# bcollico/Deep-Multiview-Depth-Estimation

Hardware: AMD Instinct MI355X
Metric: depth maps/sec + warp-kernel HBM GB/s, 3-view 640x512 D=192, 1/2/4/8 GPU (higher is better)
Workload: dtype f32

## Files before the change

deep-multiview-depth-estimation_amd/csrc/conv3d_narrow.hip:

```cpp
#include <algorithm>

#include "launchers.h"
#include "packed.h"

namespace mvs {
namespace {

constexpr int kTX = 32, kTY = 8, kDT = 4;

struct Head1 {
  const float* w1p;
  const float *sc, *sh, *mu;
  float* y1;
  int o0[3], on[3];
  int pad[3];
};

#ifndef MVS_HEAD_WAVES
#define MVS_HEAD_WAVES 3
#endif

template <int COUT, int C4, bool WZ = false, int DT = kDT, bool FOLD = false, bool C1 = false>
__global__ __launch_bounds__(kBlock) __attribute__((amdgpu_waves_per_eu(C1 ? MVS_HEAD_WAVES : 1)))
void conv3d_k3_narrow_kernel(
    const float* __restrict__ in, const float* __restrict__ wt, float* __restrict__ out, int Cin,
    int D, int H, int W, int tiles_x, int tiles_y, int dgroups, int n_batch, const float* __restrict__ bn_scale,
    const float* __restrict__ bn_shift, const float* __restrict__ bn_mean, const float* __restrict__ in2,
    const float* __restrict__ ibn, Head1 h1) {
  static_assert(!FOLD || (COUT == 1 && C4 == 0), "folded input BN: conv_out on NCDHW");
  static_assert(!WZ || DT == 4, "depth Winograd: two windows of 2");
  static_assert(!C1 || (COUT == 8 && C4 == 1 && WZ), "fused conv_1_0: the fp32 conv_0_0 kernel");
  constexpr int kPX = kTX + 2, kPY = kTY + 2, kPD = DT + 2;
  constexpr int kPlane = kPX * kPY;
  constexpr int kStage = kPD * kPlane;
  constexpr int kPer = (kStage + kBlock - 1) / kBlock;
  constexpr int NP = COUT / 2;
  constexpr int NQ = C4 ? 4 : 1;
  __shared__ float lds[NQ * kStage];
  __shared__ __attribute__((aligned(16))) float w1s[C1 ? 27 * 16 * 4 : 4];
  const int total = (int)gridDim.x;
  int t = xcd_work_id((int)blockIdx.x, total);
  if (t >= tiles_x * tiles_y * dgroups * n_batch) return;
  const int tx0 = (t % tiles_x) * kTX;
  t /= tiles_x;
  const int ty0 = (t % tiles_y) * kTY;
  t /= tiles_y;
  const int d0 = (t % dgroups) * DT;
  const int b = t / dgroups;
  const size_t plane = (size_t)H * W;
  const size_t vol = (size_t)D * plane;
  const float* ib = in + (size_t)b * Cin * vol;
  const uint2* ib16 = reinterpret_cast<const uint2*>(reinterpret_cast<const char*>(in) + (size_t)b * Cin * vol * 2);

  int goff[kPer];
  bool gok[kPer];
#pragma unroll
  for (int j = 0; j < kPer; ++j) {
    const int e = (int)threadIdx.x + j * kBlock;
    const int pd = e / kPlane, r = e % kPlane;
    const int py = r / kPX, px = r % kPX;
    const int gz = d0 + pd - 1, gy = ty0 + py - 1, gx = tx0 + px - 1;
    gok[j] = e < kStage && gz >= 0 && gz < D && gy >= 0 && gy < H && gx >= 0 && gx < W;
    goff[j] = gok[j] ? (int)((size_t)gz * plane + (size_t)gy * W + gx) : 0;
  }
  float pre[kPer][NQ];
  float pre2[FOLD ? kPer : 1];
  const float* ib2 = FOLD ? in2 + (size_t)b * Cin * vol : nullptr;
  auto fetch = [&](int q) {
    if constexpr (C4 == 2) {
      const uint2* src = ib16 + (size_t)q * vol;
#pragma unroll
      for (int j = 0; j < kPer; ++j) {
        const uint2 v = gok[j] ? src[goff[j]] : make_uint2(0u, 0u);
        pre[j][0] = __uint_as_float(v.x << 16);
        pre[j][1] = __uint_as_float(v.x & 0xFFFF0000u);
        pre[j][2] = __uint_as_float(v.y << 16);
        pre[j][3] = __uint_as_float(v.y & 0xFFFF0000u);
      }
    } else if constexpr (C4) {
      const float4* src = reinterpret_cast<const float4*>(ib) + (size_t)q * vol;
#pragma unroll
      for (int j = 0; j < kPer; ++j) {
        const float4 v = gok[j] ? src[goff[j]] : make_float4(0.0f, 0.0f, 0.0f, 0.0f);
        pre[j][0] = v.x;
        pre[j][1] = v.y;
        pre[j][2] = v.z;
        pre[j][3] = v.w;
      }
    } else {
      const float* src = ib + (size_t)q * vol;
#pragma unroll
      for (int j = 0; j < kPer; ++j) pre[j][0] = gok[j] ? src[goff[j]] : 0.0f;
      if constexpr (FOLD) {
        const float* src2 = ib2 + (size_t)q * vol;
#pragma unroll
        for (int j = 0; j < kPer; ++j) pre2[j] = gok[j] ? src2[goff[j]] : 0.0f;
      }
    }
  };
  fetch(0);

  const int lx = (int)threadIdx.x % kTX, ly = (int)threadIdx.x / kTX;
  f2v acc2[DT][NP > 0 ? NP : 1];
  float acc1[DT];
#pragma unroll
  for (int d = 0; d < DT; ++d) {
    acc1[d] = 0.0f;
#pragma unroll
    for (int q = 0; q < (NP > 0 ? NP : 1); ++q) acc2[d][q] = f2v{0.0f, 0.0f};
  }
  f2v accw[WZ ? 2 : 1][WZ ? 4 : 1][WZ ? NP : 1];
  if constexpr (WZ) {
#pragma unroll
    for (int a = 0; a < 2; ++a)
#pragma unroll
      for (int ps = 0; ps < 4; ++ps)
#pragma unroll
        for (int q = 0; q < NP; ++q) accw[a][ps][q] = f2v{0.0f, 0.0f};
  }
  const int c1lane = (int)threadIdx.x & 63, c1wave = (int)threadIdx.x >> 6;
  const int m16 = c1lane & 15, kq = c1lane >> 4;
  f4v c1acc[2] = {f4v{0.0f, 0.0f, 0.0f, 0.0f}, f4v{0.0f, 0.0f, 0.0f, 0.0f}};
  int abase[2] = {0, 0};
  if constexpr (C1) {
#pragma unroll
    for (int rb = 0; rb < 2; ++rb) {
      const int rbi = 2 * c1wave + rb, wy = rbi & 3, wzz = rbi >> 2;
      abase[rb] = kq * kStage + (2 * wzz) * kPlane + (2 * wy) * kPX + 2 * m16;
    }
  }

  const int passes = C4 ? Cin / 4 : Cin;
  for (int q = 0; q < passes; ++q) {
    __syncthreads();
    if constexpr (FOLD) {
      const float sa = ibn[q], ha = ibn[Cin + q], ma = ibn[2 * Cin + q];
      const float sb = ibn[3 * Cin + q], hb = ibn[4 * Cin + q], mb = ibn[5 * Cin + q];
#pragma unroll
      for (int j = 0; j < kPer; ++j)
        if (gok[j]) pre[j][0] = fmaxf((pre[j][0] - ma) * sa + ha, 0.0f) + fmaxf((pre2[j] - mb) * sb + hb, 0.0f);
    }
#pragma unroll
    for (int j = 0; j < kPer; ++j) {
      const int e = (int)threadIdx.x + j * kBlock;
      if (e < kStage)
#pragma unroll
        for (int u = 0; u < NQ; ++u) lds[u * kStage + e] = pre[j][u];
    }
    if constexpr (C1) {
      const f4v* src = reinterpret_cast<const f4v*>(h1.w1p) + (size_t)q * 432;
      f4v* dst = reinterpret_cast<f4v*>(w1s);
      for (int i = (int)threadIdx.x; i < 432; i += kBlock) dst[i] = src[i];
    }
    __syncthreads();
    if (q + 1 < passes) fetch(q + 1);
#pragma unroll 1
    for (int u = 0; u < NQ; ++u) {
      const int c = q * NQ + u;
      const float* lc = lds + u * kStage;
      if constexpr (WZ) {
#pragma unroll
        for (int ky = 0; ky < 3; ++ky)
#pragma unroll
          for (int kx = 0; kx < 3; ++kx) {
            float t[kPD];
#pragma unroll
            for (int p = 0; p < kPD; ++p) t[p] = lc[p * kPlane + (ly + ky) * kPX + lx + kx];
            const f2v z0 = {t[0], t[2]}, z1 = {t[1], t[3]}, z2 = {t[2], t[4]}, z3 = {t[3], t[5]};
            const f2v v[4] = {z0 - z2, z1 + z2, z2 - z1, z1 - z3};
            asm volatile("" ::: "memory");
            const f2v* wg = reinterpret_cast<const f2v*>(wt + ((size_t)(c * 9 + ky * 3 + kx) * 4) * 8);
#pragma unroll
            for (int ps = 0; ps < 4; ++ps)
#pragma unroll
              for (int qq = 0; qq < NP; ++qq) {
                const f2v u = wg[ps * 4 + qq];
                accw[0][ps][qq] = __builtin_elementwise_fma(f2v{v[ps].x, v[ps].x}, u, accw[0][ps][qq]);
                accw[1][ps][qq] = __builtin_elementwise_fma(f2v{v[ps].y, v[ps].y}, u, accw[1][ps][qq]);
              }
          }
        continue;
      }
      float tap[kPD][3][3];
#pragma unroll
      for (int p = 0; p < kPD; ++p)
#pragma unroll
        for (int ry = 0; ry < 3; ++ry)
#pragma unroll
          for (int kx = 0; kx < 3; ++kx) tap[p][ry][kx] = lc[p * kPlane + (ly + ry) * kPX + lx + kx];
#pragma unroll
      for (int kd = 0; kd < 3; ++kd) {
        if constexpr (COUT == 8) {
#pragma unroll
          for (int qq = 0; qq < NP; ++qq) {
            asm volatile("" ::: "memory");
            const f2v* wg = reinterpret_cast<const f2v*>(wt + ((size_t)(c * 3 + kd) * 9) * 8) + qq;
            f2v wp[9];
#pragma unroll
            for (int k = 0; k < 9; ++k) wp[k] = wg[k * 4];
#pragma unroll
            for (int d = 0; d < DT; ++d)
#pragma unroll
              for (int ky = 0; ky < 3; ++ky)
#pragma unroll
                for (int kx = 0; kx < 3; ++kx) {
                  const float tv = tap[d + kd][ky][kx];
                  acc2[d][qq] = __builtin_elementwise_fma(f2v{tv, tv}, wp[ky * 3 + kx], acc2[d][qq]);
                }
          }
        } else {
          asm volatile("" ::: "memory");
          const float* wg = wt + ((size_t)c * 3 + kd) * 9;
          float w9[9];
#pragma unroll
          for (int k = 0; k < 9; ++k) w9[k] = wg[k];
#pragma unroll
          for (int d = 0; d < DT; ++d)
#pragma unroll
            for (int ky = 0; ky < 3; ++ky)
#pragma unroll
              for (int kx = 0; kx < 3; ++kx) acc1[d] = fmaf(tap[d + kd][ky][kx], w9[ky * 3 + kx], acc1[d]);
        }
      }
    }
    if constexpr (C1) {
#pragma unroll
      for (int t = 0; t < 27; ++t) {
        const int tz = t / 9, ty = (t / 3) % 3, tx = t % 3;
        const float bv = w1s[t * 64 + m16 * 4 + kq];
#pragma unroll
        for (int rb = 0; rb < 2; ++rb)
          c1acc[rb] = __builtin_amdgcn_mfma_f32_16x16x4f32(lds[abase[rb] + tz * kPlane + ty * kPX + tx], bv,
                                                           c1acc[rb], 0, 0, 0);
      }
    }
  }

  if constexpr (C1) {
    const float sc = h1.sc ? h1.sc[m16] : 1.0f, sh = h1.sc ? h1.sh[m16] : 0.0f, mu = h1.sc ? h1.mu[m16] : 0.0f;
#pragma unroll
    for (int rb = 0; rb < 2; ++rb) {
      const int rbi = 2 * c1wave + rb, wy = rbi & 3, wzz = rbi >> 2;
      const int oz = (d0 - 1 + 2 * wzz + h1.pad[0]) >> 1, oy = (ty0 - 1 + 2 * wy + h1.pad[1]) >> 1;
      if (oz < h1.o0[0] || oz >= h1.o0[0] + h1.on[0] || oy < h1.o0[1] || oy >= h1.o0[1] + h1.on[1]) continue;
#pragma unroll
      for (int r = 0; r < 4; ++r) {
        const int ox = (tx0 - 1 + 2 * (4 * kq + r) + h1.pad[2]) >> 1;
        if (ox < h1.o0[2] || ox >= h1.o0[2] + h1.on[2]) continue;
        float v = c1acc[rb][r];
        if (h1.sc) v = fmaxf((v - mu) * sc + sh, 0.0f);
        h1.y1[((((size_t)b * h1.on[0] + (oz - h1.o0[0])) * h1.on[1] + (oy - h1.o0[1])) * h1.on[2] + (ox - h1.o0[2])) *
                  16 + m16] = v;
      }
    }
  }

  if constexpr (WZ) {
#pragma unroll
    for (int a = 0; a < 2; ++a)
#pragma unroll
      for (int qq = 0; qq < NP; ++qq) {
        acc2[2 * a][qq] = accw[a][0][qq] + accw[a][1][qq] + accw[a][2][qq];
        acc2[2 * a + 1][qq] = accw[a][1][qq] - accw[a][2][qq] - accw[a][3][qq];
      }
  }
  const int gx = tx0 + lx, gy = ty0 + ly;
  if (gx >= W || gy >= H) return;
  float* ob = out + (size_t)b * COUT * vol + (size_t)gy * W + gx;
#pragma unroll
  for (int d = 0; d < DT; ++d) {
    if (d0 + d >= D) break;
#pragma unroll
    for (int co = 0; co < COUT; ++co) {
      float v = COUT == 8 ? acc2[d][co / 2][co & 1] : acc1[d];
      if (bn_scale) v = fmaxf((v - bn_mean[co]) * bn_scale[co] + bn_shift[co], 0.0f);
      ob[(size_t)co * vol + (size_t)(d0 + d) * plane] = v;
    }
  }
}

#ifndef MVS_CONV_OUT_DT
#define MVS_CONV_OUT_DT 8
#endif
constexpr int kOutDT = MVS_CONV_OUT_DT;

template <int COUT, int C4, bool WZ = false, bool FOLD = false, bool C1 = false>
void launch_narrow(const float* in, const float* weight, float* out, int B, int Cin, int D, int H, int W,
                   const float* bn_scale, const float* bn_shift, const float* bn_mean, hipStream_t s,
                   const float* in2 = nullptr, const float* ibn = nullptr, const Head1& h1 = Head1{}) {
  constexpr int DT = COUT == 1 ? kOutDT : kDT;
  const int tiles_x = (W + kTX - 1) / kTX, tiles_y = (H + kTY - 1) / kTY, dgroups = (D + DT - 1) / DT;
  const dim3 grid = xcd_grid(B * dgroups * tiles_y * tiles_x);
  hipLaunchKernelGGL((conv3d_k3_narrow_kernel<COUT, C4, WZ, DT, FOLD, C1>), grid, dim3(kBlock), 0, s, in, weight,
                     out, Cin, D, H, W, tiles_x, tiles_y, dgroups, B, bn_scale, bn_shift, bn_mean, in2, ibn, h1);
}

}

void launch_conv3d_k3_narrow(const float* in, int in_c4, bool wino_z, const float* weight, float* out, int B,
                             int Cin, int Cout, int D, int H, int W, const float* bn_scale, const float* bn_shift,
                             const float* bn_mean, hipStream_t s, const float* in2, const float* ibn) {
  if (ibn) {
    launch_narrow<1, 0, false, true>(in, weight, out, B, Cin, D, H, W, bn_scale, bn_shift, bn_mean, s, in2, ibn);
    return;
  }
#define MVS_NARROW(CO, Q, WZ) launch_narrow<CO, Q, WZ>(in, weight, out, B, Cin, D, H, W, bn_scale, bn_shift, bn_mean, s)
  if (wino_z) {
    if (in_c4 == 2) MVS_NARROW(8, 2, true);
    else if (in_c4) MVS_NARROW(8, 1, true);
    else MVS_NARROW(8, 0, true);
  } else if (Cout == 8) {
    if (in_c4 == 2) MVS_NARROW(8, 2, false);
    else if (in_c4) MVS_NARROW(8, 1, false);
    else MVS_NARROW(8, 0, false);
  } else {
    if (in_c4 == 2) MVS_NARROW(1, 2, false);
    else if (in_c4) MVS_NARROW(1, 1, false);
    else MVS_NARROW(1, 0, false);
  }
#undef MVS_NARROW
}

void launch_conv_head_fp32(const float* cv4, int B, int D, int H, int W, const float* w0wz, const float* bn0_sc,
                           const float* bn0_sh, const float* bn0_mu, const float* w1, const float* w1p,
                           const float* bn1_sc, const float* bn1_sh, const float* bn1_mu, const int* pad,
                           const int* o0, const int* on, float* y0, float* y1, hipStream_t s, hipEvent_t ev0,
                           hipEvent_t ev1) {
  Head1 h1;
  h1.w1p = w1p;
  h1.sc = bn1_sc;
  h1.sh = bn1_sh;
  h1.mu = bn1_mu;
  h1.y1 = y1;
  for (int d = 0; d < 3; ++d) {
    h1.o0[d] = o0[d];
    h1.on[d] = on[d];
    h1.pad[d] = pad[d];
  }
  if (ev0) (void)hipEventRecord(ev0, s);
  launch_narrow<8, 1, true, false, true>(cv4, w0wz, y0, B, 32, D, H, W, bn0_sc, bn0_sh, bn0_mu, s, nullptr, nullptr,
                                         h1);
  if (ev1) (void)hipEventRecord(ev1, s);
  const int tile[3] = {kDT, kTY, kTX}, n[3] = {D, H, W};
  int clo[3], chi[3];
  for (int d = 0; d < 3; ++d) {
    const int tiles = (n[d] + tile[d] - 1) / tile[d];
    clo[d] = std::max(o0[d], (pad[d] - 1) / 2);
    chi[d] = std::min(o0[d] + on[d] - 1, (tiles * tile[d] - 3 + pad[d]) / 2);
  }
  for (int d = 0; d < 3; ++d)
    for (int side = 0; side < 2; ++side) {
      int so[3], sn[3];
      bool empty = false;
      for (int e = 0; e < 3; ++e) {
        if (e < d) {
          so[e] = clo[e];
          sn[e] = chi[e] - clo[e] + 1;
        } else if (e > d) {
          so[e] = o0[e];
          sn[e] = on[e];
        } else if (side == 0) {
          so[e] = o0[e];
          sn[e] = clo[e] - o0[e];
        } else {
          so[e] = chi[e] + 1;
          sn[e] = o0[e] + on[e] - 1 - chi[e];
        }
        empty = empty || sn[e] <= 0;
      }
      if (empty) continue;
      int st0[3];
      for (int e = 0; e < 3; ++e) st0[e] = so[e] - o0[e];
      launch_conv3d_region(1 , false, 1, cv4, nullptr, w1, y1, B, 32, 16, n, so, sn, nullptr, nullptr, pad,
                           bn1_sc, bn1_sh, bn1_mu, s, nullptr, nullptr, false, st0, on);
    }
}

}
```

Before: 677.1.

## Precompute depth-Winograd input transform into LDS with column-per-thread staging

For the depth-Winograd (WZ, non-C1) narrow conv path, each thread now loads a full depth column of the halo tile and applies the Winograd input transform once before storing to LDS as packed float4 tiles. The inner 3x3 loop then reads two float4 values per tap instead of six scalars plus redundant add/subtract. This removes repeated transforms and LDS reads across the channels and taps. The cost is a different LDS layout, more registers for the column prefetch, and uneven work for the threads handling the leftover columns.

Result: faster. 684.0 (median of 6 runs) (+1.0%).

```diff
diff --git a/deep-multiview-depth-estimation_amd/csrc/conv3d_narrow.hip b/deep-multiview-depth-estimation_amd/csrc/conv3d_narrow.hip
--- a/deep-multiview-depth-estimation_amd/csrc/conv3d_narrow.hip
+++ b/deep-multiview-depth-estimation_amd/csrc/conv3d_narrow.hip
@@ -36,7 +36,11 @@
   constexpr int kPer = (kStage + kBlock - 1) / kBlock;
   constexpr int NP = COUT / 2;
   constexpr int NQ = C4 ? 4 : 1;
-  __shared__ float lds[NQ * kStage];
+  constexpr bool TILE = WZ && !C1;
+  constexpr int kRest = kPlane - kBlock, LS = C4 ? 2 : 1, NR = NQ / LS;
+  static_assert(kRest > 0 && kRest * LS <= kBlock, "one column per thread and one part of the rest");
+  constexpr int kTile = NQ * kPlane * 4;
+  __shared__ __attribute__((aligned(16))) float lds[TILE ? 2 * kTile : NQ * kStage];
   __shared__ __attribute__((aligned(16))) float w1s[C1 ? 27 * 16 * 4 : 4];
   const int total = (int)gridDim.x;
   int t = xcd_work_id((int)blockIdx.x, total);
@@ -52,10 +56,21 @@
   const float* ib = in + (size_t)b * Cin * vol;
   const uint2* ib16 = reinterpret_cast<const uint2*>(reinterpret_cast<const char*>(in) + (size_t)b * Cin * vol * 2);
 
+  auto column = [&](int e, bool use, int& off) {
+    const int gy = ty0 + e / kPX - 1, gx = tx0 + e % kPX - 1;
+    const bool ok = use && gy >= 0 && gy < H && gx >= 0 && gx < W;
+    off = ok ? gy * W + gx : 0;
+    return ok;
+  };
+  const int col2 = kBlock + (int)threadIdx.x % kRest, part2 = (int)threadIdx.x / kRest;
+  int coff = 0, coff2 = 0;
+  const bool cok = TILE && column((int)threadIdx.x, true, coff);
+  const bool cok2 = TILE && column(col2, part2 < LS, coff2);
+  float prec[TILE ? kPD : 1][NQ], prec2[TILE ? kPD : 1][NR];
   int goff[kPer];
   bool gok[kPer];
 #pragma unroll
-  for (int j = 0; j < kPer; ++j) {
+  for (int j = 0; j < (TILE ? 0 : kPer); ++j) {
     const int e = (int)threadIdx.x + j * kBlock;
     const int pd = e / kPlane, r = e % kPlane;
     const int py = r / kPX, px = r % kPX;
@@ -67,7 +82,37 @@
   float pre2[FOLD ? kPer : 1];
   const float* ib2 = FOLD ? in2 + (size_t)b * Cin * vol : nullptr;
   auto fetch = [&](int q) {
-    if constexpr (C4 == 2) {
+    if constexpr (TILE) {
+#pragma unroll
+      for (int p = 0; p < kPD; ++p) {
+        const int gz = d0 + p - 1;
+        const bool zok = gz >= 0 && gz < D;
+        const size_t zo = (size_t)q * vol + (zok ? (size_t)gz * plane : 0);
+        if constexpr (C4 == 2) {
+          const uint2 v = cok && zok ? ib16[zo + coff] : make_uint2(0u, 0u);
+          prec[p][0] = __uint_as_float(v.x << 16);
+          prec[p][1] = __uint_as_float(v.x & 0xFFFF0000u);
+          prec[p][2] = __uint_as_float(v.y << 16);
+          prec[p][3] = __uint_as_float(v.y & 0xFFFF0000u);
+          const uint32_t r = cok2 && zok ? reinterpret_cast<const uint32_t*>(ib16 + zo + coff2)[part2] : 0u;
+          prec2[p][0] = __uint_as_float(r << 16);
+          prec2[p][1] = __uint_as_float(r & 0xFFFF0000u);
+        } else if constexpr (C4) {
+          const float4* src = reinterpret_cast<const float4*>(ib) + zo;
+          const float4 v = cok && zok ? src[coff] : make_float4(0.0f, 0.0f, 0.0f, 0.0f);
+          prec[p][0] = v.x;
+          prec[p][1] = v.y;
+          prec[p][2] = v.z;
+          prec[p][3] = v.w;
+          const float2 r = cok2 && zok ? reinterpret_cast<const float2*>(src + coff2)[part2] : make_float2(0.0f, 0.0f);
+          prec2[p][0] = r.x;
+          prec2[p][1] = r.y;
+        } else {
+          prec[p][0] = cok && zok ? ib[zo + coff] : 0.0f;
+          prec2[p][0] = cok2 && zok ? ib[zo + coff2] : 0.0f;
+        }
+      }
+    } else if constexpr (C4 == 2) {
       const uint2* src = ib16 + (size_t)q * vol;
 #pragma unroll
       for (int j = 0; j < kPer; ++j) {
@@ -140,12 +185,36 @@
       for (int j = 0; j < kPer; ++j)
         if (gok[j]) pre[j][0] = fmaxf((pre[j][0] - ma) * sa + ha, 0.0f) + fmaxf((pre2[j] - mb) * sb + hb, 0.0f);
     }
-#pragma unroll
-    for (int j = 0; j < kPer; ++j) {
-      const int e = (int)threadIdx.x + j * kBlock;
-      if (e < kStage)
-#pragma unroll
-        for (int u = 0; u < NQ; ++u) lds[u * kStage + e] = pre[j][u];
+    if constexpr (TILE) {
+      auto put = [&](const float (&z)[kPD], int u, int e) {
+        f4v* ta = reinterpret_cast<f4v*>(lds) + u * kPlane + e;
+        ta[0] = f4v{z[0] - z[2], z[1] + z[2], z[2] - z[1], z[1] - z[3]};
+        ta[kTile / 4] = f4v{z[2] - z[4], z[3] + z[4], z[4] - z[3], z[3] - z[5]};
+      };
+#pragma unroll
+      for (int u = 0; u < NQ; ++u) {
+        float z[kPD];
+#pragma unroll
+        for (int p = 0; p < kPD; ++p) z[p] = prec[p][u];
+        put(z, u, (int)threadIdx.x);
+      }
+      if (part2 < LS) {
+#pragma unroll
+        for (int u = 0; u < NR; ++u) {
+          float z[kPD];
+#pragma unroll
+          for (int p = 0; p < kPD; ++p) z[p] = prec2[p][u];
+          put(z, part2 * NR + u, col2);
+        }
+      }
+    } else {
+#pragma unroll
+      for (int j = 0; j < kPer; ++j) {
+        const int e = (int)threadIdx.x + j * kBlock;
+        if (e < kStage)
+#pragma unroll
+          for (int u = 0; u < NQ; ++u) lds[u * kStage + e] = pre[j][u];
+      }
     }
     if constexpr (C1) {
       const f4v* src = reinterpret_cast<const f4v*>(h1.w1p) + (size_t)q * 432;
@@ -157,17 +226,28 @@
 #pragma unroll 1
     for (int u = 0; u < NQ; ++u) {
       const int c = q * NQ + u;
-      const float* lc = lds + u * kStage;
+      const float* lc = lds + (TILE ? 0 : u * kStage);
       if constexpr (WZ) {
 #pragma unroll
         for (int ky = 0; ky < 3; ++ky)
 #pragma unroll
           for (int kx = 0; kx < 3; ++kx) {
-            float t[kPD];
-#pragma unroll
-            for (int p = 0; p < kPD; ++p) t[p] = lc[p * kPlane + (ly + ky) * kPX + lx + kx];
-            const f2v z0 = {t[0], t[2]}, z1 = {t[1], t[3]}, z2 = {t[2], t[4]}, z3 = {t[3], t[5]};
-            const f2v v[4] = {z0 - z2, z1 + z2, z2 - z1, z1 - z3};
+            f2v v[4];
+            if constexpr (TILE) {
+              const f4v* ta = reinterpret_cast<const f4v*>(lds) + u * kPlane + (ly + ky) * kPX + lx + kx;
+              const f4v va = ta[0], vb = ta[kTile / 4];
+#pragma unroll
+              for (int ps = 0; ps < 4; ++ps) v[ps] = f2v{va[ps], vb[ps]};
+            } else {
+              float t[kPD];
+#pragma unroll
+              for (int p = 0; p < kPD; ++p) t[p] = lc[p * kPlane + (ly + ky) * kPX + lx + kx];
+              const f2v z0 = {t[0], t[2]}, z1 = {t[1], t[3]}, z2 = {t[2], t[4]}, z3 = {t[3], t[5]};
+              v[0] = z0 - z2;
+              v[1] = z1 + z2;
+              v[2] = z2 - z1;
+              v[3] = z1 - z3;
+            }
             asm volatile("" ::: "memory");
             const f2v* wg = reinterpret_cast<const f2v*>(wt + ((size_t)(c * 9 + ky * 3 + kx) * 4) * 8);
 #pragma unroll
```
